# szemenyeim/DynEnv

Measured on AMD Instinct MI355X. Metric: agent-steps/s, higher is better.
Workload: dtype f64

## Files before the change

### dynenv_amd/csrc/driving_kernels.hip

```cpp
#include "driving_dev.h"

__constant__ DrvConst C;

#include "driving_host.h"

struct DrvMailbox {
  double p1x[DRV_NS][2], p1y[DRV_NS][2], p2x[DRV_NS][2], p2y[DRV_NS][2], nx[DRV_NS], ny[DRV_NS];
  int hash[DRV_NS][2], count[DRV_NS], flag[DRV_NS];
};
struct DrvObsStage {
  float carRow[DRV_MAXA][8];
  float goal[DRV_MAXA][2];
  float shared[DRV_MAXO * 4 + DRV_MAXP * 2 + DRV_LANE_ROWS * 5];
};
#ifdef DRV_PROFILE
#define DRV_PROF(...) __VA_ARGS__
#else
#define DRV_PROF(...)
#endif
#define DRV_CLIST 128
struct __align__(16) DrvLds {
  double px[DRV_NB], py[DRV_NB], vx[DRV_NB], vy[DRV_NB], ang[DRV_NB], w[DRV_NB], vbx[DRV_NB], vby[DRV_NB], wb[DRV_NB];
  double minv[DRV_NB], iinv[DRV_NB];
  double rc[16], rs[16], rotAng[16];
  double dirx[16], diry[16], prevx[16], prevy[16], goalx[16], goaly[16];
  double cosRel0[16];
  double dprev[16];
  double cmass[16], cpower[16], chx[16], chy[16];
  double aabb[DRV_MAXA][4];
  int flags[DRV_NB], moving[DRV_NB];
  double ox[DRV_MAXO], oy[DRV_MAXO];
  int s_pair[DRV_NS], s_meta[DRV_NS], s_hash0[DRV_NS], s_hash1[DRV_NS];
  double s_jn0[DRV_NS], s_jt0[DRV_NS], s_jn1[DRV_NS], s_jt1[DRV_NS];
  double rewAcc[16], posAcc[16];
  int lastCand[64];
  int stepErr;
  unsigned char act[16];
  int still[DRV_NB];
  unsigned short clist[DRV_CLIST];
  int clistN;
  int sLvMeta;
  unsigned long long sActive;
  unsigned char sLevel[DRV_NS];
  union {
    DrvMailbox mb;
    DrvObsStage ob;
  } u;
};

static_assert(sizeof(DrvLds) <= 10240, "16 one-wave workgroups per CU - one residency round of 4096 environments on 256 CUs - need <= 160 KB / 16 of LDS each");
__shared__ DrvLds g_L;


#define CF_FIN(f) (((f) >> 4) & 1)
#define CF_CRASHED(f) (((f) >> 5) & 1)
#define CF_FRIC(f) (((f) >> 6) & 1)
#define CF_LP(f) (((f) >> 8) & 7)
#define CF_SET_LP(f, lp) (((f) & ~(7 << 8)) | ((lp) << 8))
#define CF_CRASH_BITS ((1 << 4) | (1 << 5) | (1 << 6))
#define PF_ROAD(f) ((f)&1)
#define PF_SIDE(f) (((f) >> 1) & 1)
#define PF_DEAD(f) (((f) >> 2) & 1)
#define PF_CROSSING(f) (((f) >> 3) & 1)
#define PF_BEGIN(f) (((f) >> 4) & 1)
#define PF_SPEED(f) (((f) >> 8) & 15)

#define DRV_COS_PI_2 6.123233995736766e-17
template <int R>
struct RoadK;
template <>
struct RoadK<0> {
  static constexpr double p0x = 875.0, p0y = 0.0, dirx = 0.0, diry = 1.0, lat = 2.0 * 35.0 + 5.0, length = 1000.0;
  static constexpr double dirAngle = 1.5707963267948966, cosDir0 = DRV_COS_PI_2, nx = -1.0, ny = DRV_COS_PI_2;
};
template <>
struct RoadK<1> {
  static constexpr double p0x = 0.0, p0y = 500.0, dirx = 1.0, diry = 0.0, lat = 1.0 * 35.0 + 5.0, length = 1750.0;
  static constexpr double dirAngle = 0.0, cosDir0 = 1.0, nx = DRV_COS_PI_2, ny = 1.0;
};

struct CarK {
  static constexpr double carMass0 = 1200.0, carMass1 = 1800.0, carMass2 = 3500.0, carMass3 = 5000.0;
  static constexpr double carHx0 = 10.0, carHx1 = 15.0, carHx2 = 20.0, carHx3 = 25.0;
  static constexpr double carHy0 = 5.0, carHy1 = 6.0, carHy2 = 7.0, carHy3 = 8.0;
  static constexpr double carPower0 = 3.0, carPower1 = 4.0, carPower2 = 3.0, carPower3 = 4.0;
  static constexpr double carInertia0 = 50000.0, carInertia1 = 156600.0, carInertia2 = 0x1.ff8e555555555p+18, carInertia3 = 0x1.185ad55555555p+20;
  static constexpr double pedMass = 90.0, pedInertia = 90.0 * (0.5 * (0.0 * 0.0 + 5.0 * 5.0) + 0.0);
};

template <int R>
DE_DEV int road_pos(V2 point, double cosRel) {
  V2 pt = vsub(point, v2(RoadK<R>::p0x, RoadK<R>::p0y));
  double dist = vcross(v2(RoadK<R>::dirx, RoadK<R>::diry), pt);
  if (dm_abs(dist) >= RoadK<R>::lat) return LP_OffRoad;
  int pos = LP_OverRoad;
  double dirDist = vdot(v2(RoadK<R>::dirx, RoadK<R>::diry), pt);
  if (dirDist >= -10.0 && dirDist <= RoadK<R>::length + 10.0) {
    double relAngle = cosRel * dist;
    pos = relAngle < 0.0 ? LP_InRightLane : LP_InOpposingLane;
  }
  return pos;
}

DE_DEV bool drv_is_off_road(V2 point) {
  int position = LP_OffRoad;
  int rp = road_pos<0>(point, RoadK<0>::cosDir0);
  if (rp < position) position = rp;
  rp = road_pos<1>(point, RoadK<1>::cosDir0);
  if (rp < position) position = rp;
  return position >= LP_OverRoad;
}
DE_DEV bool drv_is_out(V2 p) { return p.x <= 0.0 || p.y <= 0.0 || p.x >= DRV_W || p.y >= DRV_H; }

DE_DEV void apply_friction(double& vx, double& vy, double& w, double m, double friction, double rotFriction,
                           double spin) {
  vx = vx * 1.0 + (0.0 + 0.0) * DE_DT;
  vy = vy * 1.0 + (0.0 + 0.0) * DE_DT;
  w = w * 1.0 + 0.0;
  double factor = friction * m;
// ... 256 lines not shown
  b.w = dm_fma(b.iinv, dms_cross(r.x, r.y, j.x, j.y), b.w);
}
DE_DEV void apply_bias_impulse(BodyV& b, V2 j, V2 r) {
  b.vb = v2(dm_fma(j.x, b.minv, b.vb.x), dm_fma(j.y, b.minv, b.vb.y));
  b.wb = dm_fma(b.iinv, dms_cross(r.x, r.y, j.x, j.y), b.wb);
}
DE_DEV double bias_rel_n(const BodyV& a, const BodyV& b, V2 r1, V2 r2, V2 n) {
  const V2 vb1 = v2(dms_point_vx(a.vb.x, r1.y, a.wb), dms_point_vy(a.vb.y, r1.x, a.wb));
  const V2 vb2 = v2(dms_point_vx(b.vb.x, r2.y, b.wb), dms_point_vy(b.vb.y, r2.x, b.wb));
  return vdot_f(vsub(vb2, vb1), n);
}

#define STD_NORM_X (0.5 / (DRV_W + 100.0))
#define STD_NORM_Y (0.5 / (DRV_H + 100.0))
#define STD_NORM_W (1.0 / 15.0)
#define STD_NORM_H (1.0 / 25.0)
DE_DEV double normalize_obs(double pt, double nf, double mean) { return ((pt * nf) - mean) * 2.0 * 1.0; }

DE_DEV float obs_self_or_car(const DrvObsStage& O, int A, int a, int ff) {
  if (ff < 6) return O.carRow[a][ff];
  if (ff < 8) return O.goal[a][ff - 6];
  if (ff == 8) return O.carRow[a][6];
  int c = (ff - 9) / 7, kk = (ff - 9) - c * 7;
  c += (c >= a);
  return O.carRow[c][kk];
}

DE_OOL void write_full_obs_ool(int lane, int A, int nPed, int nObst, int obs_dim, float* __restrict__ out) {
  DrvLds& L = g_L;
  DrvObsStage& O = L.u.ob;
  __syncthreads();
  if (lane < A) {
    int f = L.flags[lane];
    O.carRow[lane][0] = (float)normalize_obs(L.px[lane], STD_NORM_X, 0.0);
    O.carRow[lane][1] = (float)normalize_obs(L.py[lane], STD_NORM_Y, 0.0);
    O.carRow[lane][2] = (float)L.rc[lane];
    O.carRow[lane][3] = (float)L.rs[lane];
    O.carRow[lane][4] = (float)normalize_obs(L.chy[lane], STD_NORM_W, 0.5);
    O.carRow[lane][5] = (float)normalize_obs(L.chx[lane], STD_NORM_H, 0.5);
    O.carRow[lane][6] = (float)CF_FIN(f);
    O.goal[lane][0] = (float)normalize_obs(L.goalx[lane], STD_NORM_X, 0.0);
    O.goal[lane][1] = (float)normalize_obs(L.goaly[lane], STD_NORM_Y, 0.0);
  }
  if (lane >= DRV_SLOT_PED && lane < DRV_SLOT_PED + DRV_MAXP) {
    int k = lane - DRV_SLOT_PED;
    bool on = k < nPed;
    O.shared[DRV_MAXO * 4 + 2 * k + 0] = on ? (float)normalize_obs(L.px[lane], STD_NORM_X, 0.0) : 0.0f;
    O.shared[DRV_MAXO * 4 + 2 * k + 1] = on ? (float)normalize_obs(L.py[lane], STD_NORM_Y, 0.0) : 0.0f;
  }
  if (lane < DRV_MAXO) {
    bool on = lane < nObst;
    O.shared[4 * lane + 0] = on ? (float)normalize_obs(L.ox[lane], STD_NORM_X, 0.0) : 0.0f;
    O.shared[4 * lane + 1] = on ? (float)normalize_obs(L.oy[lane], STD_NORM_Y, 0.0) : 0.0f;
    O.shared[4 * lane + 2] = on ? (float)normalize_obs(10.0, STD_NORM_W, 0.5) : 0.0f;
    O.shared[4 * lane + 3] = on ? (float)normalize_obs(10.0, STD_NORM_H, 0.5) : 0.0f;
  }
  if (lane < DRV_LANE_ROWS * 5) O.shared[DRV_MAXO * 4 + DRV_MAXP * 2 + lane] = C.laneRows[lane];
  __syncthreads();
  const int carsEnd = 9 + (A - 1) * 7;
  if (((carsEnd | obs_dim) & 3) == 0) {
    for (int f = lane; f < carsEnd; f += DE_WAVE) {
      const bool own = f < 9;
      const int p = own ? 0 : (f - 9) / 7, col = own ? (f < 6 ? f : (f == 8 ? 6 : f - 6)) : (f - 9) - p * 7;
      const bool fromGoal = f == 6 || f == 7;
      for (int a = 0; a < A; ++a) {
        const int k = own ? a : p + (p >= a ? 1 : 0);
        out[(size_t)a * obs_dim + f] = fromGoal ? O.goal[a][col] : O.carRow[k][col];
      }
    }
    const int nvec = (obs_dim - carsEnd) >> 2;
    for (int q = lane; q < nvec; q += DE_WAVE) {
      const float4 v = *reinterpret_cast<const float4*>(&O.shared[q << 2]);
      for (int a = 0; a < A; ++a) *reinterpret_cast<float4*>(out + (size_t)a * obs_dim + carsEnd + (q << 2)) = v;
    }
  } else {
    for (int idx = lane; idx < A * obs_dim; idx += DE_WAVE) {
      int a = idx / obs_dim, ff = idx - a * obs_dim;
      out[idx] = ff < carsEnd ? obs_self_or_car(O, A, a, ff) : O.shared[ff - carsEnd];
    }
  }
  __syncthreads();
}

DE_DEV void load_env(const DrvState& S, DrvLds& L, int e, int lane, int A, int nPed, int nObst, uint64_t occ) {
  const size_t E = (size_t)S.E;
  const int bl = lane & (DRV_NB - 1), cl = lane & 15, ol = lane < DRV_MAXO ? lane : DRV_MAXO - 1, sl = lane < DRV_NS ? lane : DRV_NS - 1;
  const double* b = S.body + (size_t)e * DRV_NB + bl;
  const double g_px = b[BF_PX * E * DRV_NB], g_py = b[BF_PY * E * DRV_NB], g_vx = b[BF_VX * E * DRV_NB], g_vy = b[BF_VY * E * DRV_NB];
  const double g_ang = b[BF_ANG * E * DRV_NB], g_w = b[BF_W * E * DRV_NB];
  const double g_vbx = b[BF_VBX * E * DRV_NB], g_vby = b[BF_VBY * E * DRV_NB], g_wb = b[BF_WB * E * DRV_NB];
  const int g_f = S.flags[(size_t)e * DRV_NB + bl], g_aux = S.aux[(size_t)e * DRV_NB + bl];
  const double* c = S.carx + (size_t)e * 16 + cl;
  const double g_prevx = c[CF_PREVX * E * 16], g_prevy = c[CF_PREVY * E * 16], g_gx = c[CF_GOALX * E * 16], g_gy = c[CF_GOALY * E * 16];
  const double g_dirx = c[CF_DIRX * E * 16], g_diry = c[CF_DIRY * E * 16];
  const double g_ox = S.obst[(size_t)e * DRV_MAXO + ol], g_oy = S.obst[E * DRV_MAXO + (size_t)e * DRV_MAXO + ol];
  int g_pair = 0xFFFF, g_meta = 0, g_h0 = 0, g_h1 = 0;
  double g_jn0 = 0.0, g_jt0 = 0.0, g_jn1 = 0.0, g_jt1 = 0.0;
  if (occ != 0ull) {
    const size_t o = (size_t)e * DRV_NS + sl;
    g_pair = S.s_pair[o]; g_meta = S.s_meta[o];
    g_h0 = (int)S.s_hash[o]; g_h1 = (int)S.s_hash[E * DRV_NS + o];
    g_jn0 = S.s_imp[o]; g_jt0 = S.s_imp[E * DRV_NS + o]; g_jn1 = S.s_imp[2 * E * DRV_NS + o]; g_jt1 = S.s_imp[3 * E * DRV_NS + o];
  }
  if (lane < DRV_NB) {
    const bool used = lane < A || (lane >= DRV_SLOT_PED && lane < DRV_SLOT_PED + nPed);
    L.px[lane] = used ? g_px : 0.0; L.py[lane] = used ? g_py : 0.0;
    L.vx[lane] = used ? g_vx : 0.0; L.vy[lane] = used ? g_vy : 0.0;
    const double ang = used ? g_ang : 0.0;
    L.ang[lane] = ang; L.w[lane] = used ? g_w : 0.0;
    L.vbx[lane] = used ? g_vbx : 0.0; L.vby[lane] = used ? g_vby : 0.0;
    L.wb[lane] = used ? g_wb : 0.0;
    const int f = used ? g_f : 0;
    L.flags[lane] = f;
    L.moving[lane] = used ? g_aux : 0;
    const int ty = f & 3;
#define DRV_BY_TYPE(ARR) (ty == 3 ? CarK::ARR##3 : (ty == 2 ? CarK::ARR##2 : (ty == 1 ? CarK::ARR##1 : CarK::ARR##0)))
    double minv = 0.0, iinv = 0.0;
    if (lane < A) { minv = 1.0 / DRV_BY_TYPE(carMass); iinv = 1.0 / DRV_BY_TYPE(carInertia); }
    else if (used) { minv = 1.0 / CarK::pedMass; iinv = 1.0 / CarK::pedInertia; }
    L.minv[lane] = minv; L.iinv[lane] = iinv;
    if (lane < 16) { L.rc[lane] = 1.0; L.rs[lane] = 0.0; L.rotAng[lane] = 0.0; }
    if (lane < A) {
      L.dirx[lane] = g_dirx; L.diry[lane] = g_diry;
      L.prevx[lane] = g_prevx; L.prevy[lane] = g_prevy; L.goalx[lane] = g_gx; L.goaly[lane] = g_gy;
      L.dprev[lane] = vlen(vsub(v2(g_prevx, g_prevy), v2(g_gx, g_gy)));
      L.cmass[lane] = DRV_BY_TYPE(carMass); L.cpower[lane] = DRV_BY_TYPE(carPower);
      L.chx[lane] = DRV_BY_TYPE(carHx); L.chy[lane] = DRV_BY_TYPE(carHy);
      car_refresh_rot(L, lane, ang);
    }
#undef DRV_BY_TYPE
  }
  if (lane < DRV_MAXO) {
    L.ox[lane] = lane < nObst ? g_ox : 0.0;
    L.oy[lane] = lane < nObst ? g_oy : 0.0;
  }
  if (lane < DRV_NS) {
    const bool on = (occ >> lane) & 1ull;
    L.s_pair[lane] = on ? g_pair : 0xFFFF;
    L.s_meta[lane] = on ? g_meta : 0;
    L.s_hash0[lane] = on ? g_h0 : 0; L.s_hash1[lane] = on ? g_h1 : 0;
    L.s_jn0[lane] = on ? g_jn0 : 0.0; L.s_jt0[lane] = on ? g_jt0 : 0.0;
    L.s_jn1[lane] = on ? g_jn1 : 0.0; L.s_jt1[lane] = on ? g_jt1 : 0.0;
  }
}

DE_DEV void store_env(const DrvState& S, const DrvLds& L, int e, int lane, int A, int nPed, uint64_t occ) {
  const size_t E = (size_t)S.E;
  if (lane < A || (lane >= DRV_SLOT_PED && lane < DRV_SLOT_PED + nPed)) {
    double* b = S.body + (size_t)e * DRV_NB + lane;
    b[BF_PX * E * DRV_NB] = L.px[lane]; b[BF_PY * E * DRV_NB] = L.py[lane]; b[BF_VX * E * DRV_NB] = L.vx[lane];
    b[BF_VY * E * DRV_NB] = L.vy[lane]; b[BF_ANG * E * DRV_NB] = L.ang[lane]; b[BF_W * E * DRV_NB] = L.w[lane];
    b[BF_VBX * E * DRV_NB] = L.vbx[lane]; b[BF_VBY * E * DRV_NB] = L.vby[lane]; b[BF_WB * E * DRV_NB] = L.wb[lane];
    S.flags[(size_t)e * DRV_NB + lane] = L.flags[lane];
    if (lane < A) {
      double* c = S.carx + (size_t)e * 16 + lane;
      c[CF_DIRX * E * 16] = L.dirx[lane]; c[CF_DIRY * E * 16] = L.diry[lane];
      c[CF_PREVX * E * 16] = L.prevx[lane]; c[CF_PREVY * E * 16] = L.prevy[lane];
    } else {
      S.aux[(size_t)e * DRV_NB + lane] = L.moving[lane];
    }
  }
  if (lane < DRV_NS && ((occ >> lane) & 1ull)) {
    size_t o = (size_t)e * DRV_NS + lane;
    S.s_pair[o] = L.s_pair[lane]; S.s_meta[o] = L.s_meta[lane];
    S.s_hash[o] = (uint32_t)L.s_hash0[lane]; S.s_hash[E * DRV_NS + o] = (uint32_t)L.s_hash1[lane];
    S.s_imp[o] = L.s_jn0[lane]; S.s_imp[E * DRV_NS + o] = L.s_jt0[lane];
    S.s_imp[2 * E * DRV_NS + o] = L.s_jn1[lane]; S.s_imp[3 * E * DRV_NS + o] = L.s_jt1[lane];
  }
}

DE_DEV bool cb_begin(DrvLds& L, int i, int j, int lane) {
  const double v1x = L.vx[i], v1y = L.vy[i];
  const int f1 = L.flags[i];
  if (j < DRV_SLOT_PED) {
    const double v2x = L.vx[j], v2y = L.vy[j];
    const int f2 = L.flags[j];
    const int crashed1 = CF_CRASHED(f1), crashed2 = CF_CRASHED(f2), pos1 = CF_LP(f1), pos2 = CF_LP(f2);
    const double v1len = vlen(v2(v1x, v1y)), v2len = vlen(v2(v2x, v2y));
    const double v1l = v1len / 5.0, v2l = v2len / 5.0;
    double r1 = L.rewAcc[i], r2 = L.rewAcc[j];
    if (!crashed1) r1 -= v1l;
    if (!crashed2) r2 -= v2l;
    if (pos1 != LP_InRightLane && !crashed1) r1 -= v1l;
    if (pos2 != LP_InRightLane && !crashed2) r2 -= v2l;
    if (pos1 == LP_InRightLane && pos2 == LP_InRightLane) {
      V2 dp = v2(L.px[i] - L.px[j], L.py[i] - L.py[j]);
      double adp = dev_atan2(dp.y, dp.x);
      if (v1len > 1.0 && dev_cos(adp - dev_atan2(v1y, v1x)) < -0.4 && !crashed1) r1 -= v1l;
      if (v2len > 1.0 && dev_cos(adp - dev_atan2(v2y, v2x)) > 0.4 && !crashed2) r2 -= v2l;
    }
    if (lane == i) { L.rewAcc[i] = r1; L.flags[i] = f1 | CF_CRASH_BITS; }
    if (lane == j) { L.rewAcc[j] = r2; L.flags[j] = f2 | CF_CRASH_BITS; }
    return true;
  } else if (j < DRV_SLOT_OBST) {
    const double v1l = vlen(v2(v1x, v1y));
    if (v1l > 1.0) {
      V2 dp = v2(L.px[i] - L.px[j], L.py[i] - L.py[j]);
      if (lane == j) {
        L.moving[j] = 0; L.vx[j] = 0.0; L.vy[j] = 0.0; L.flags[j] = L.flags[j] | (1 << 2);
      }
      if (dev_cos(dev_atan2(dp.y, dp.x) - dev_atan2(v1y, v1x)) < -0.4 && !CF_FIN(f1)) {
        if (lane == i) { L.flags[i] = f1 | CF_CRASH_BITS; L.rewAcc[i] = L.rewAcc[i] - v1l / 5.0; }
      }
      return true;
    }
    return false;
  } else {
    if (lane == i) {
      if (!CF_FIN(f1)) L.rewAcc[i] = L.rewAcc[i] - vlen(v2(v1x, v1y)) / 5.0;
      L.flags[i] = f1 | CF_CRASH_BITS;
    }
    return true;
  }
}

DE_DEV void arb_warm_start(BodyV& a, BodyV& b, V2 n, const V2* r1, const V2* r2, const double* jn, const double* jt,
                           int count) {
#pragma unroll
  for (int c = 0; c < 2; ++c) {
    if (c == 0 || count > 1) {
      V2 j = vrotate_f(n, v2(jn[c], jt[c]));
      j = vmul(j, 1.0);
      apply_impulse(a, vneg(j), r1[c]);
      apply_impulse(b, j, r2[c]);
    }
  }
// ... 758 lines not shown
            const V2 nv = vmul(vmul(dir, (double)PF_SPEED(f)), (double)speed);
            vx = nv.x; vy = nv.y;
          } else if (isOffRoad) {
            crossing = 0; beginc = 0;
          }
        }
        L.moving[lane] = moving;
        L.flags[lane] = PEDF_PACK(PF_ROAD(f), side, 0, crossing, beginc, PF_SPEED(f));
        L.vx[lane] = vx; L.vy[lane] = vy;
      }
    }

DRV_PROF(const unsigned long long Q3 = __builtin_amdgcn_s_memtime();)
    double bl = 0.0, bb = 0.0, br = -1.0, bt = -1.0;
    bool live = false;
    int sj = 3;
    if (isBody) {
      const double npx = px + (vx + vbx) * DE_DT, npy = py + (vy + vby) * DE_DT, nang = ang + (w + wb) * DE_DT;
      const bool still = !turned && vx == 0.0 && vy == 0.0 && w == 0.0 && vbx == 0.0 && vby == 0.0 && wb == 0.0;
      L.px[lane] = npx; L.py[lane] = npy; L.ang[lane] = nang;
      const bool frozen = !turned && vx == 0.0 && vy == 0.0 && w == 0.0 && npx == px && npy == py && nang == ang;
      sj = (still ? 1 : 0) | (frozen ? 2 : 0);
      L.still[lane] = sj;
      live = true;
      if (isCar) {
        if (nang != rotAngv) { const CarRot cr = car_refresh_rot<true>(L, lane, nang); rcv = cr.c; rsv = cr.s; }
        if (!aabbValid || !frozen) {
          BoxW bw;
          box_world(bw, v2(npx, npy), rcv, rsv, chx, chy);
          double l = INFINITY, r = -INFINITY, b = INFINITY, t = -INFINITY;
#pragma unroll
          for (int k = 0; k < 4; ++k) {
            l = fmin_cp(l, bw.v[k].x); r = fmax_cp(r, bw.v[k].x); b = fmin_cp(b, bw.v[k].y); t = fmax_cp(t, bw.v[k].y);
          }
          bl = l - 0.0; bb = b - 0.0; br = r + 0.0; bt = t + 0.0;
          L.aabb[lane][0] = bl; L.aabb[lane][1] = bb; L.aabb[lane][2] = br; L.aabb[lane][3] = bt;
        } else {
          bl = L.aabb[lane][0]; bb = L.aabb[lane][1]; br = L.aabb[lane][2]; bt = L.aabb[lane][3];
        }
      } else {
        bl = npx - 5.0; bb = npy - 5.0; br = npx + 5.0; bt = npy + 5.0;
      }
    } else if (lane >= DRV_SLOT_OBST && lane < DRV_SLOT_BLD + 4) {
      live = lane >= DRV_SLOT_BLD || (lane - DRV_SLOT_OBST) < nObst;
      const V2 c = static_pos(L, lane);
      const double ex = lane >= DRV_SLOT_BLD ? 400.0 : 10.0, ey = lane >= DRV_SLOT_BLD ? 225.0 : 10.0;
      bl = -ex + c.x; br = ex + c.x; bb = -ey + c.y; bt = ey + c.y;
    }
    aabbValid = true;
    __syncthreads();
DRV_PROF(const unsigned long long Q4 = __builtin_amdgcn_s_memtime();)

    int cand = 0;
    bool candMoving = false, removed = false;
    int dirty = 0;
    {
      const int carStill = (int)(wave_ballot(isCar && (sj & 1)) & 0x3FFull);
      const int carFrozen = (int)(wave_ballot(isCar && (sj & 2)) & 0x3FFull);
#pragma unroll
      for (int i = 0; i < DRV_MAXA; ++i) {
        const double al = L.aabb[i][0], ab = L.aabb[i][1], ar = L.aabb[i][2], at = L.aabb[i][3];
        const bool hit = (al <= br) & (bl <= ar) & (ab <= bt) & (bb <= at);
        cand |= hit ? (1 << i) : 0;
      }
      {
        const int lim = lane < A ? lane : A;
        cand &= live ? ((1 << lim) - 1) : 0;
      }
      if (cand) candMoving = !(sj & 1) || (cand & ~carStill) != 0;
      const int clean = (lastCand >= 0 && (sj & 2)) ? (cand & lastCand & carFrozen) : 0;
      dirty = cand & ~clean;
      removed = lastCand < 0 || (lastCand & ~cand) != 0;
    }
  L.lastCand[lane] = cand;
DRV_PROF(if (lane == 0 && blockIdx.x < 4096) { unsigned long long* d = g_dbgl + blockIdx.x * 8; const unsigned long long Q5 = __builtin_amdgcn_s_memtime(); if (it == 0) { for (int k = 0; k < 8; ++k) d[k] = 0ull; } d[0] += Q1 - Q0; d[1] += Q2 - Q1; d[2] += Q3 - Q2; d[3] += Q4 - Q3; d[4] += Q5 - Q4; d[5] += Q5 - Q0; })
  DrvLightRet ret;
  ret.cand = cand; ret.dirty = dirty; ret.bits = (candMoving ? 1 : 0) | (removed ? 2 : 0) | (cand != lastCand ? 4 : 0);
  return ret;
}
DE_DEV unsigned drv_hw_simd_key() {
  const unsigned hw = (unsigned)__builtin_amdgcn_s_getreg(63492) , xcc = (unsigned)__builtin_amdgcn_s_getreg(63508) ;
  return ((xcc & 0xFu) << 16) | (hw & 0xFF30u);
}
DE_DEV int drv_launch_tick(const DrvState& S) { return S.tick_src ? uniform_i(__atomic_load_n(&S.iso[13], __ATOMIC_RELAXED)) : S.tick; }
DE_DEV int drv_launch_pv(const DrvState& S) { return S.tick_src ? uniform_i(__atomic_load_n(&S.iso[14], __ATOMIC_RELAXED)) : S.pv_par; }
DE_DEV int drv_iso_assign(const DrvState& S, int lane, int tick) {
  const int b = blockIdx.x, E = S.E;
  if (!S.iso_on) return b;
  const int buf = tick % 3;
  if (b == 0 && lane == 0) { const int nn = (tick + 2) % 3; S.iso[nn] = 0; S.iso[3 + nn] = 0; }
  if (S.iso_on == 3) return b;
  int K = uniform_i(S.iso[buf]);
  const int cap = S.iso_on == 1 ? DRV_ISO_MAX : DRV_ISO_LIST;
  K = K < cap ? K : cap;
  const int G = S.iso_on == 1 ? 4 * DRV_ISO_GROUPS : E;
  if (S.iso_on == 1) {
    if (b < G) { if (lane == 0) S.iso_hw[(size_t)(tick & 1) * (4 * DRV_ISO_GROUPS) + b] = drv_hw_simd_key(); }
    else if (b == G + 3 * DRV_ISO_MAX) {
      const unsigned* hw = S.iso_hw + (size_t)((tick + 1) & 1) * (4 * DRV_ISO_GROUPS);
      bool bad = false;
      for (int g = DRV_ISO_G0 + lane; g < DRV_ISO_G0 + DRV_ISO_GSPAN; g += 64) {
        const unsigned k0 = hw[g], k1 = hw[g + DRV_ISO_GROUPS], k2 = hw[g + 2 * DRV_ISO_GROUPS], k3 = hw[g + 3 * DRV_ISO_GROUPS];
        bad |= k0 == 0xFFFFFFFFu || k0 != k1 || k0 != k2 || k0 != k3;
      }
      const bool ok = wave_ballot(bad) == 0ull;
      if (lane == 0) {
        int cd = S.iso[12];
        if (!ok) cd = DRV_ISO_COOLDOWN; else if (cd > 0) cd -= 1;
        S.iso[12] = cd;
        S.iso[8 + (tick + 1) % 3] = (ok && cd == 0) ? 1 : 0;
        if (!ok && tick > 1) atomicAdd(&S.iso[11], 1);
      }
      return -1;
    }
    if (uniform_i(S.iso[8 + buf]) != 1) K = 0;
  }
  if (K == 0) return b < E ? b : -1;
  const int* H = S.iso + DRV_ISO_HDR + buf * DRV_ISO_LIST;
  int r;
  if (S.iso_on == 2) {
    if (b < K) return uniform_i(H[b]);
    r = b - K;
  } else if (b >= G) {
    const int d = b - G;
    if (d >= 3 * K) return -1;
    r = (G - 4 * K) + d;
  } else {
    const int g = b & (DRV_ISO_GROUPS - 1), pos = b / DRV_ISO_GROUPS;
    if ((unsigned)(g - DRV_ISO_G0) < (unsigned)K) {
      const int h = uniform_i(H[g - DRV_ISO_G0]);
      if (pos == 0) return h;
      int i = 0;
      for (; i < 96; ++i) {
        if (uniform_i(__atomic_load_n(&S.iso_done[h], __ATOMIC_RELAXED)) == tick) break;
        __builtin_amdgcn_s_sleep(127);
      }
      if (i >= 96 && lane == 0) atomicAdd(&S.iso[7], 1);
      return -1;
    }
    r = pos * (DRV_ISO_GROUPS - K) + (g < DRV_ISO_G0 ? g : g - K);
  }
  int h0 = 0x7FFFFFFF, h1 = h0, h2 = h0, h3 = h0;
  if (lane < K) h0 = H[lane];
  if (lane + 64 < K) h1 = H[lane + 64];
  if (lane + 128 < K) h2 = H[lane + 128];
  if (lane + 192 < K) h3 = H[lane + 192];
  int x = r;
  for (int it = 0; it <= DRV_ISO_LIST; ++it) {
    const int c = __popcll(wave_ballot(h0 <= x)) + __popcll(wave_ballot(h1 <= x)) + __popcll(wave_ballot(h2 <= x)) + __popcll(wave_ballot(h3 <= x));
    const int nx = r + c;
    if (nx == x) break;
    x = nx;
  }
  return x < E ? x : -1;
}
#ifndef DRV_ISO_MIN
#define DRV_ISO_MIN 300000
#endif
#ifndef DRV_ISO_PCT
#define DRV_ISO_PCT 75
#endif
DE_DEV void drv_iso_report(const DrvState& S, int e, int lane, unsigned long long t0, int tick) {
  if (!S.iso_on || lane != 0) return;
  const int cycles = (int)(__builtin_amdgcn_s_memtime() - t0);
  const int buf = tick % 3, nxt = (tick + 1) % 3;
  const int slowest = S.iso[3 + buf];
  if (cycles > DRV_ISO_MIN && cycles > (slowest / 100) * DRV_ISO_PCT) atomicMax(&S.iso[3 + nxt], cycles);
  if (S.iso_on == 3) return;
  if (slowest > DRV_ISO_MIN && cycles > (slowest / 100) * DRV_ISO_PCT) {
    const int k = atomicAdd(&S.iso[nxt], 1);
    if (k < DRV_ISO_LIST) S.iso[DRV_ISO_HDR + nxt * DRV_ISO_LIST + k] = e;
  }
  __atomic_store_n(&S.iso_done[e], tick, __ATOMIC_RELAXED);
}

template <bool PARTIAL>
DE_DEV void drv_step_body(const DrvState& S, const int* __restrict__ actions, float* __restrict__ obs, double* __restrict__ rewards,
                          uint8_t* __restrict__ dones, float* __restrict__ pobs, int pvNoise, double pvMagn) {
  const unsigned long long isoT0 = __builtin_amdgcn_s_memtime();
DRV_PROF(const unsigned long long KS = isoT0;)
  DrvLds& L = g_L;
  int lane = threadIdx.x;
  const int tick = drv_launch_tick(S);
  if (!S.tick_src && blockIdx.x == 0 && lane == 0) { S.iso[13] = S.tick; S.iso[14] = S.pv_par; }
  const int e = drv_iso_assign(S, lane, tick);
  if (e < 0) return;
DRV_PROF(if (lane < 8 && e < 4096) { g_dbgp[e * 8 + lane] = 0ull; g_dbgs[e * 8 + lane] = 0ull; })
  const int A = S.A;
  int* envi = S.envi + (size_t)e * EI_COUNT;
  int elapsed = uniform_i(envi[EI_ELAPSED]);
  int allFinished = uniform_i(envi[EI_ALLFIN]);
  const int nPed = uniform_i(envi[EI_NPED]);
  const int nObst = uniform_i(envi[EI_NOBST]);
  const uint32_t episode = (uint32_t)uniform_i(envi[EI_EPISODE]);
  uint64_t occ = (uint64_t)(uint32_t)uniform_i(envi[EI_OCC]);
  if (occ != 0ull) __builtin_amdgcn_s_setprio(3);
  else if (PARTIAL) __builtin_amdgcn_s_setprio(1);
  const uint32_t genv = (uint32_t)(S.env_id_offset + e);

  const bool isCar = lane < A;
  const bool isPed = lane >= DRV_SLOT_PED && lane < DRV_SLOT_PED + nPed;
  const bool isBody = isCar || isPed;
  const int g_act0 = actions[((size_t)e * A + (isCar ? lane : 0)) * 2 + 0], g_act1 = actions[((size_t)e * A + (isCar ? lane : 0)) * 2 + 1];
  const int g_lastCand = S.lastcand[(size_t)e * 64 + lane];
  load_env(S, L, e, lane, A, nPed, nObst, occ);

  {
    int act0 = isCar ? g_act0 : 1, act1 = isCar ? g_act1 : 1;
    const bool bad = (unsigned)act0 > 2u || (unsigned)act1 > 2u;
    if (bad) { act0 = 1; act1 = 1; }
    if (lane < 16) L.act[lane] = (unsigned char)(act0 | (act1 << 2));
    const bool anyBad = wave_ballot(bad) != 0ull;
    if (lane == 0) L.stepErr = anyBad ? 2 : 0;
  }
  int finishedAt = -1;
  if (lane < 16) { L.rewAcc[lane] = 0.0; L.posAcc[lane] = 0.0; }
  bool aabbValid = false;
  L.lastCand[lane] = g_lastCand;
  if (lane == 0) { L.clistN = -1; L.sActive = ~0ull; L.sLvMeta = 0; }
  bool inertAll = (uniform_i(envi[EI_PAD]) & 1) != 0;
  bool steadyAll = (uniform_i(envi[EI_PAD]) & 2) != 0;
  bool vbValid = (uniform_i(envi[EI_PAD]) & 4) != 0;
  int nFast = 0, nQuiet = 0, nContact = 0, nSlots = 0, nWhyCand = 0, nWhyMoving = 0, nWhyInert = 0, nSteady = 0, nLight = 0, nSplit = 0;
  __syncthreads();

DRV_PROF(const unsigned long long K0 = __builtin_amdgcn_s_memtime(); unsigned long long tPh1 = 0, tBroad = 0, tFast = 0, tCont = 0, tBook = 0;)
  bool lightOff = false;
  for (int it = 0; it < 10; ++it) {
    lane = fresh_lane();
DRV_PROF(const unsigned long long A0 = __builtin_amdgcn_s_memtime();)
    const DrvLightRet lr = drv_light_substep(it, lane, A, nPed, nObst, elapsed, (uint32_t)S.seed, (uint32_t)(S.seed >> 32), genv, episode,
                                             (vbValid ? 1 : 0) | (aabbValid ? 2 : 0));
    const int cand = lr.cand, dirty = lr.dirty;
    const bool candMoving = (lr.bits & 1) != 0, removed = (lr.bits & 2) != 0;
    aabbValid = true;
DRV_PROF(const unsigned long long A1 = A0;)
    const uint64_t anyCand = wave_ballot(cand != 0);
    const bool candChanged = wave_ballot((lr.bits & 4) != 0) != 0ull, anyMoving = wave_ballot(candMoving) != 0ull;
    if (candChanged && lane == 0) L.clistN = -1;
    const bool quiescent = inertAll && !candChanged && !anyMoving;
    const bool steadyOk = !quiescent && steadyAll && wave_ballot(removed) == 0ull;
    const bool anyDirty = wave_ballot(dirty != 0) != 0ull;
    bool replay = steadyOk && !anyDirty;
    const bool light = steadyOk && anyDirty && !lightOff;
    if (!(anyCand == 0ull && occ == 0ull) && !quiescent && !replay) { if (candChanged) nWhyCand++; else if (anyMoving) nWhyMoving++; else nWhyInert++; }

DRV_PROF(const unsigned long long A2 = __builtin_amdgcn_s_memtime(); bool tookContact = false;)
    if (anyCand == 0ull && occ == 0ull) nFast++; else if (quiescent) nQuiet++; else if (replay) nSteady++; else nContact++;
    nSlots += __popcll(occ);
    if ((anyCand == 0ull && occ == 0ull) || quiescent) {
      velocity_update_ool(A | (nPed << 8));
      if (anyCand == 0ull && occ == 0ull) steadyAll = false;
      vbValid = false;
    } else if (!replay) {
DRV_PROF(tookContact = true;)
      __builtin_amdgcn_s_setprio(3);
      ContactRet cr = drv_contact_path(lane, cand, dirty, light ? 1 : 0, A, A | (nPed << 8), occ);
      lane = fresh_lane();
      if (wave_ballot((cr.err & 1) != 0) != 0ull && lane == 0) L.stepErr |= 1;
      if (light && !(uniform_i(cr.err >> 3) & 1)) lightOff = true;
      if (uniform_i(cr.err >> 3) & 1) {
        replay = true; nLight++;
      } else {
        nSplit += uniform_i(cr.err >> 4) & 1;
        occ = uniform_u64(cr.occ);
        inertAll = (uniform_i(cr.err >> 1) & 1) != 0;
        steadyAll = (uniform_i(cr.err >> 2) & 1) != 0;
        vbValid = true;
      }
    }
    if (replay) {
      velocity_update_ool(A | (nPed << 8));
      vbValid = true;
    }
    __syncthreads();

DRV_PROF(const unsigned long long A3 = __builtin_amdgcn_s_memtime(); tPh1 += A1 - A0; tBroad += A2 - A1; if (tookContact) tCont += A3 - A2; else tFast += A3 - A2;)
    elapsed += 1;
    bool notDone = false;
    if (isCar) { int f = L.flags[lane]; notDone = !(CF_FIN(f) && !CF_CRASHED(f)); }
    const bool allFin = wave_ballot(notDone) == 0ull;
    if (!allFinished && allFin) {
      allFinished = 1;
      finishedAt = elapsed;
    }
  }
  lane = fresh_lane();
  const double teamReward = finishedAt >= 0 ? 0.0 + (double)(DRV_MAX_TIME - finishedAt) / 100.0 : 0.0;

DRV_PROF(const unsigned long long K1 = __builtin_amdgcn_s_memtime();)
  double* er = S.epr + (size_t)e * 16 + (isCar ? lane : 0);
  double* ep = S.epr + (size_t)S.E * 16 + (size_t)e * 16 + (isCar ? lane : 0);
  const double g_er = *er, g_ep = *ep;
  const int cl = lane < 10 ? lane : 0;
  const int g_cnt = envi[EI_N_FAST + cl];
  const int g_err = envi[EI_ERR];
  double rew = 0.0, posrew = 0.0;
  if (isCar) {
    rew = L.rewAcc[lane] + teamReward;
    posrew = L.posAcc[lane] + dm_max(0.0, teamReward);
    rewards[(size_t)e * A + lane] = rew;
  }
  if (lane == 0) {
    dones[e] = (uint8_t)(elapsed >= DRV_MAX_TIME);
    envi[EI_ELAPSED] = elapsed; envi[EI_ALLFIN] = allFinished; envi[EI_OCC] = (int)(uint32_t)occ;
    envi[EI_PAD] = (inertAll ? 1 : 0) | (steadyAll ? 2 : 0) | (vbValid ? 4 : 0);
  }
  const int errBits = uniform_i(L.stepErr);
  S.lastcand[(size_t)e * 64 + lane] = L.lastCand[lane];
  store_env(S, L, e, lane, A, nPed, occ);
  if (obs) write_full_obs_ool(lane, A, nPed, nObst, S.obs_dim, obs + (size_t)e * A * S.obs_dim);
  if (isCar) { *er = g_er + rew; *ep = g_ep + posrew; }
  {
    static_assert(EI_N_QUIET == EI_N_FAST + 1 && EI_N_CONTACT == EI_N_FAST + 2 && EI_N_SLOTS == EI_N_FAST + 3 && EI_N_WHY_CAND == EI_N_FAST + 4 &&
                  EI_N_WHY_MOVING == EI_N_FAST + 5 && EI_N_WHY_INERT == EI_N_FAST + 6 && EI_N_STEADY == EI_N_FAST + 7 && EI_N_LIGHT == EI_N_FAST + 8 && EI_N_SPLIT == EI_N_FAST + 9,
                  "the diagnostic counters are consecutive");
    const int add = lane == 0 ? nFast : lane == 1 ? nQuiet : lane == 2 ? nContact : lane == 3 ? nSlots : lane == 4 ? nWhyCand : lane == 5 ? nWhyMoving :
                    lane == 6 ? nWhyInert : lane == 7 ? nSteady : lane == 8 ? nLight : nSplit;
    if (lane < 10) envi[EI_N_FAST + lane] = g_cnt + add;
  }
  if (errBits && lane == 0) envi[EI_ERR] = g_err | errBits;
  int fusedAgents = !(PARTIAL && pobs) ? 0 : nContact >= DRV_DEFER_MIN_CONTACT ? 0 : (A < DRV_FUSED_AGENTS ? A : DRV_FUSED_AGENTS);
  int budget = 0;
  if (PARTIAL && pobs && S.iso_on >= 2) {
    const int slowest = uniform_i(S.iso[3 + tick % 3]);
    if (slowest > 0) {
      budget = (slowest / 100) * DRV_PV_DEADLINE_PCT - (int)(__builtin_amdgcn_s_memtime() - isoT0);
      fusedAgents = budget > 0 ? A : 0;
    }
  }
  drv_iso_report(S, e, fresh_lane(), isoT0, tick);
  if (PARTIAL && fusedAgents > 0) {
    __builtin_amdgcn_s_setprio(0);
    PvIn in;
    in.px = in.py = in.ang = in.ox = in.oy = in.gx = in.gy = 0.0; in.flags = 0;
    if (lane < DRV_NB && (lane < A || (lane >= DRV_SLOT_PED && lane < DRV_SLOT_PED + nPed))) {
      in.px = L.px[lane]; in.py = L.py[lane]; in.ang = L.ang[lane]; in.flags = L.flags[lane];
    }
    if (lane < nObst) { in.ox = L.ox[lane]; in.oy = L.oy[lane]; }
    if (lane < A) { in.gx = L.goalx[lane]; in.gy = L.goaly[lane]; }
    fusedAgents = drv_partial_obs_fused(in, S.seed, S.A, S.envi, S.env_id_offset, e, nPed | (nObst << 8), elapsed, episode, pvNoise | (fusedAgents << 8), pvMagn,
                                        pobs, budget);
  }
  if (PARTIAL && fresh_lane() == 0) {
    envi[EI_DEFER_OBS] = fusedAgents;
    if (pobs && fusedAgents < A) {
      const int pv = drv_launch_pv(S);
      const int k = atomicAdd(&S.pvq[16 * pv], 1);
      if (k < S.E) S.pvq[32 + pv * S.E + k] = e;
      else envi[EI_ERR] = envi[EI_ERR] | 4;
    }
  }
DRV_PROF(if (lane == 0 && e < 4096) { unsigned long long* d = g_dbgw + e * 12; const unsigned long long KE = __builtin_amdgcn_s_memtime(); d[0] = KE - KS; d[1] = nContact; d[2] = __popcll(occ); d[3] = nSteady + nQuiet; d[4] = K0 - KS; d[5] = tPh1; d[6] = tBroad; d[7] = tFast; d[8] = tCont; d[9] = (K1 - K0) - tPh1 - tBroad - tFast - tCont; d[10] = KE - K1; d[11] = ((unsigned long long)__builtin_amdgcn_s_getreg(63508) << 32) | (unsigned long long)__builtin_amdgcn_s_getreg(63492); })
}

extern "C" __global__ void drv_tick_advance_kernel(DrvState S, int flipPv) {
  if (threadIdx.x == 0 && blockIdx.x == 0) { S.iso[13] = (S.iso[13] + 1) % (3 * (1 << 28)); if (flipPv) S.iso[14] = S.iso[14] ^ 1; }
}

extern "C" __global__ void __launch_bounds__(64, DRV_WAVES_PER_SIMD)
drv_step_kernel(DrvState S, const int* __restrict__ actions, float* __restrict__ obs, double* __restrict__ rewards,
                uint8_t* __restrict__ dones) {
  drv_step_body<false>(S, actions, obs, rewards, dones, nullptr, 0, 0.0);
}
extern "C" __global__ void __launch_bounds__(64, DRV_WAVES_PER_SIMD)
drv_step_partial_kernel(DrvState S, const int* __restrict__ actions, double* __restrict__ rewards, uint8_t* __restrict__ dones,
                        float* __restrict__ pobs, int pvNoise, double pvMagn) {
  drv_step_body<true>(S, actions, nullptr, rewards, dones, pobs, pvNoise, pvMagn);
}

extern "C" __global__ void __launch_bounds__(64) drv_obs_kernel(DrvState S, float* __restrict__ obs) {
  DrvLds& L = g_L;
  const int e = blockIdx.x, lane = threadIdx.x, A = S.A;
  const int* envi = S.envi + (size_t)e * EI_COUNT;
  const int nPed = uniform_i(envi[EI_NPED]), nObst = uniform_i(envi[EI_NOBST]);
  load_env(S, L, e, lane, A, nPed, nObst, 0ull);
  write_full_obs_ool(lane, A, nPed, nObst, S.obs_dim, obs + (size_t)e * A * S.obs_dim);
}

DE_DEV void road_get_spot(const DrvRoad& r, int lane, int spot, V2& pos, double& angle) {
  int end = lane >= r.nLanes ? 1 : 0;
  V2 p = end ? r.p1 : r.p0;
  V2 spotDir = vmul(end ? vneg(r.dir) : r.dir, r.followDist);
  V2 laneDir = vmul(end ? r.normal : vneg(r.normal), r.width);
  double l = (double)(end ? lane - r.nLanes : lane) + 0.5;
  pos = vadd(vadd(p, vmul(laneDir, l)), vmul(spotDir, (double)spot));
  angle = dm_atan2(spotDir.y, spotDir.x);
}
DE_DEV V2 road_get_walk_spot(const DrvRoad& r, int side, double length, double width) {
  V2 w0 = r.walk[side][0], w1 = r.walk[side][1];
  V2 center = vadd(w0, vmul(vsub(w1, w0), length));
  double f = width * r.width;
  V2 off = vmul(vmul(r.normal, f), side ? 1.0 : -1.0);
  return vadd(center, off);
}

extern "C" __global__ void __launch_bounds__(64) drv_reset_kernel(DrvState S) {
  const int e = blockIdx.x * blockDim.x + threadIdx.x;
  if (e >= S.E) return;
  const size_t E = (size_t)S.E;
  const int A = S.A;
  int* envi = S.envi + (size_t)e * EI_COUNT;
  const uint32_t ep = (uint32_t)envi[EI_EPISODE];
  const uint32_t genv = (uint32_t)(S.env_id_offset + e);
  for (int k = 0; k < DRV_NB; ++k) {
    for (int f = 0; f < BF_COUNT; ++f) S.body[(size_t)f * E * DRV_NB + (size_t)e * DRV_NB + k] = 0.0;
    S.flags[(size_t)e * DRV_NB + k] = 0;
    S.aux[(size_t)e * DRV_NB + k] = 0;
  }
  for (int k = 0; k < 16; ++k) {
    for (int f = 0; f < CF_COUNT; ++f) S.carx[(size_t)f * E * 16 + (size_t)e * 16 + k] = 0.0;
    S.epr[(size_t)e * 16 + k] = 0.0;
    S.epr[E * 16 + (size_t)e * 16 + k] = 0.0;
  }
// ... 211 lines not shown
```

Measured before the change: 261.7 million.

## Batch kernel-entry global loads and broadcast iso header via readlane

The kernel prologue now issues every per-environment global load (envi words, actions, lastcand, body/car/obstacle/slot state) up front in one batch behind a sched_barrier, instead of many dependent uniform loads. Scalars are then pulled out with readlane. The iso scheduling header and work lists are loaded once per lane and broadcast, replacing repeated scalar global reads, and the slowest-time value is cached in LDS for later use. This aims to cut serialized load latency at wave start, at the cost of more live registers and loading slot data even when it is unoccupied.

Measured after the change: 260.5 million. No clear change (-0.4%).

```diff
diff --git a/dynenv_amd/csrc/driving_kernels.hip b/dynenv_amd/csrc/driving_kernels.hip
--- a/dynenv_amd/csrc/driving_kernels.hip
+++ b/dynenv_amd/csrc/driving_kernels.hip
@@ -35,6 +35,7 @@
   double rewAcc[16], posAcc[16];
   int lastCand[64];
   int stepErr;
+  int isoSlowest;
   unsigned char act[16];
   int still[DRV_NB];
   unsigned short clist[DRV_CLIST];
@@ -457,37 +458,41 @@
   __syncthreads();
 }
 
-DE_DEV void load_env(const DrvState& S, DrvLds& L, int e, int lane, int A, int nPed, int nObst, uint64_t occ) {
+struct DrvEnvLoads {
+  double px, py, vx, vy, ang, w, vbx, vby, wb, prevx, prevy, gx, gy, dirx, diry, ox, oy, jn0, jt0, jn1, jt1;
+  int f, aux, pair, meta, h0, h1;
+};
+DE_DEV DrvEnvLoads drv_env_loads(const DrvState& S, int e, int lane) {
   const size_t E = (size_t)S.E;
   const int bl = lane & (DRV_NB - 1), cl = lane & 15, ol = lane < DRV_MAXO ? lane : DRV_MAXO - 1, sl = lane < DRV_NS ? lane : DRV_NS - 1;
+  DrvEnvLoads g;
   const double* b = S.body + (size_t)e * DRV_NB + bl;
-  const double g_px = b[BF_PX * E * DRV_NB], g_py = b[BF_PY * E * DRV_NB], g_vx = b[BF_VX * E * DRV_NB], g_vy = b[BF_VY * E * DRV_NB];
-  const double g_ang = b[BF_ANG * E * DRV_NB], g_w = b[BF_W * E * DRV_NB];
-  const double g_vbx = b[BF_VBX * E * DRV_NB], g_vby = b[BF_VBY * E * DRV_NB], g_wb = b[BF_WB * E * DRV_NB];
-  const int g_f = S.flags[(size_t)e * DRV_NB + bl], g_aux = S.aux[(size_t)e * DRV_NB + bl];
+  g.px = b[BF_PX * E * DRV_NB]; g.py = b[BF_PY * E * DRV_NB]; g.vx = b[BF_VX * E * DRV_NB]; g.vy = b[BF_VY * E * DRV_NB];
+  g.ang = b[BF_ANG * E * DRV_NB]; g.w = b[BF_W * E * DRV_NB];
+  g.vbx = b[BF_VBX * E * DRV_NB]; g.vby = b[BF_VBY * E * DRV_NB]; g.wb = b[BF_WB * E * DRV_NB];
+  g.f = S.flags[(size_t)e * DRV_NB + bl]; g.aux = S.aux[(size_t)e * DRV_NB + bl];
   const double* c = S.carx + (size_t)e * 16 + cl;
-  const double g_prevx = c[CF_PREVX * E * 16], g_prevy = c[CF_PREVY * E * 16], g_gx = c[CF_GOALX * E * 16], g_gy = c[CF_GOALY * E * 16];
-  const double g_dirx = c[CF_DIRX * E * 16], g_diry = c[CF_DIRY * E * 16];
-  const double g_ox = S.obst[(size_t)e * DRV_MAXO + ol], g_oy = S.obst[E * DRV_MAXO + (size_t)e * DRV_MAXO + ol];
-  int g_pair = 0xFFFF, g_meta = 0, g_h0 = 0, g_h1 = 0;
-  double g_jn0 = 0.0, g_jt0 = 0.0, g_jn1 = 0.0, g_jt1 = 0.0;
-  if (occ != 0ull) {
-    const size_t o = (size_t)e * DRV_NS + sl;
-    g_pair = S.s_pair[o]; g_meta = S.s_meta[o];
-    g_h0 = (int)S.s_hash[o]; g_h1 = (int)S.s_hash[E * DRV_NS + o];
-    g_jn0 = S.s_imp[o]; g_jt0 = S.s_imp[E * DRV_NS + o]; g_jn1 = S.s_imp[2 * E * DRV_NS + o]; g_jt1 = S.s_imp[3 * E * DRV_NS + o];
-  }
+  g.prevx = c[CF_PREVX * E * 16]; g.prevy = c[CF_PREVY * E * 16]; g.gx = c[CF_GOALX * E * 16]; g.gy = c[CF_GOALY * E * 16];
+  g.dirx = c[CF_DIRX * E * 16]; g.diry = c[CF_DIRY * E * 16];
+  g.ox = S.obst[(size_t)e * DRV_MAXO + ol]; g.oy = S.obst[E * DRV_MAXO + (size_t)e * DRV_MAXO + ol];
+  const size_t o = (size_t)e * DRV_NS + sl;
+  g.pair = S.s_pair[o]; g.meta = S.s_meta[o];
+  g.h0 = (int)S.s_hash[o]; g.h1 = (int)S.s_hash[E * DRV_NS + o];
+  g.jn0 = S.s_imp[o]; g.jt0 = S.s_imp[E * DRV_NS + o]; g.jn1 = S.s_imp[2 * E * DRV_NS + o]; g.jt1 = S.s_imp[3 * E * DRV_NS + o];
+  return g;
+}
+DE_DEV void drv_env_fill(DrvLds& L, const DrvEnvLoads& g, int lane, int A, int nPed, int nObst, uint64_t occ) {
   if (lane < DRV_NB) {
     const bool used = lane < A || (lane >= DRV_SLOT_PED && lane < DRV_SLOT_PED + nPed);
-    L.px[lane] = used ? g_px : 0.0; L.py[lane] = used ? g_py : 0.0;
-    L.vx[lane] = used ? g_vx : 0.0; L.vy[lane] = used ? g_vy : 0.0;
-    const double ang = used ? g_ang : 0.0;
-    L.ang[lane] = ang; L.w[lane] = used ? g_w : 0.0;
-    L.vbx[lane] = used ? g_vbx : 0.0; L.vby[lane] = used ? g_vby : 0.0;
-    L.wb[lane] = used ? g_wb : 0.0;
-    const int f = used ? g_f : 0;
+    L.px[lane] = used ? g.px : 0.0; L.py[lane] = used ? g.py : 0.0;
+    L.vx[lane] = used ? g.vx : 0.0; L.vy[lane] = used ? g.vy : 0.0;
+    const double ang = used ? g.ang : 0.0;
+    L.ang[lane] = ang; L.w[lane] = used ? g.w : 0.0;
+    L.vbx[lane] = used ? g.vbx : 0.0; L.vby[lane] = used ? g.vby : 0.0;
+    L.wb[lane] = used ? g.wb : 0.0;
+    const int f = used ? g.f : 0;
     L.flags[lane] = f;
-    L.moving[lane] = used ? g_aux : 0;
+    L.moving[lane] = used ? g.aux : 0;
     const int ty = f & 3;
 #define DRV_BY_TYPE(ARR) (ty == 3 ? CarK::ARR##3 : (ty == 2 ? CarK::ARR##2 : (ty == 1 ? CarK::ARR##1 : CarK::ARR##0)))
     double minv = 0.0, iinv = 0.0;
@@ -496,9 +501,9 @@
     L.minv[lane] = minv; L.iinv[lane] = iinv;
     if (lane < 16) { L.rc[lane] = 1.0; L.rs[lane] = 0.0; L.rotAng[lane] = 0.0; }
     if (lane < A) {
-      L.dirx[lane] = g_dirx; L.diry[lane] = g_diry;
-      L.prevx[lane] = g_prevx; L.prevy[lane] = g_prevy; L.goalx[lane] = g_gx; L.goaly[lane] = g_gy;
-      L.dprev[lane] = vlen(vsub(v2(g_prevx, g_prevy), v2(g_gx, g_gy)));
+      L.dirx[lane] = g.dirx; L.diry[lane] = g.diry;
+      L.prevx[lane] = g.prevx; L.prevy[lane] = g.prevy; L.goalx[lane] = g.gx; L.goaly[lane] = g.gy;
+      L.dprev[lane] = vlen(vsub(v2(g.prevx, g.prevy), v2(g.gx, g.gy)));
       L.cmass[lane] = DRV_BY_TYPE(carMass); L.cpower[lane] = DRV_BY_TYPE(carPower);
       L.chx[lane] = DRV_BY_TYPE(carHx); L.chy[lane] = DRV_BY_TYPE(carHy);
       car_refresh_rot(L, lane, ang);
@@ -506,17 +511,21 @@
 #undef DRV_BY_TYPE
   }
   if (lane < DRV_MAXO) {
-    L.ox[lane] = lane < nObst ? g_ox : 0.0;
-    L.oy[lane] = lane < nObst ? g_oy : 0.0;
+    L.ox[lane] = lane < nObst ? g.ox : 0.0;
+    L.oy[lane] = lane < nObst ? g.oy : 0.0;
   }
   if (lane < DRV_NS) {
     const bool on = (occ >> lane) & 1ull;
-    L.s_pair[lane] = on ? g_pair : 0xFFFF;
-    L.s_meta[lane] = on ? g_meta : 0;
-    L.s_hash0[lane] = on ? g_h0 : 0; L.s_hash1[lane] = on ? g_h1 : 0;
-    L.s_jn0[lane] = on ? g_jn0 : 0.0; L.s_jt0[lane] = on ? g_jt0 : 0.0;
-    L.s_jn1[lane] = on ? g_jn1 : 0.0; L.s_jt1[lane] = on ? g_jt1 : 0.0;
-  }
+    L.s_pair[lane] = on ? g.pair : 0xFFFF;
+    L.s_meta[lane] = on ? g.meta : 0;
+    L.s_hash0[lane] = on ? g.h0 : 0; L.s_hash1[lane] = on ? g.h1 : 0;
+    L.s_jn0[lane] = on ? g.jn0 : 0.0; L.s_jt0[lane] = on ? g.jt0 : 0.0;
+    L.s_jn1[lane] = on ? g.jn1 : 0.0; L.s_jt1[lane] = on ? g.jt1 : 0.0;
+  }
+}
+
+DE_DEV void load_env(const DrvState& S, DrvLds& L, int e, int lane, int A, int nPed, int nObst, uint64_t occ) {
+  drv_env_fill(L, drv_env_loads(S, e, lane), lane, A, nPed, nObst, occ);
 }
 
 DE_DEV void store_env(const DrvState& S, const DrvLds& L, int e, int lane, int A, int nPed, uint64_t occ) {
@@ -1441,15 +1450,30 @@
   const unsigned hw = (unsigned)__builtin_amdgcn_s_getreg(63492) , xcc = (unsigned)__builtin_amdgcn_s_getreg(63508) ;
   return ((xcc & 0xFu) << 16) | (hw & 0xFF30u);
 }
-DE_DEV int drv_launch_tick(const DrvState& S) { return S.tick_src ? uniform_i(__atomic_load_n(&S.iso[13], __ATOMIC_RELAXED)) : S.tick; }
 DE_DEV int drv_launch_pv(const DrvState& S) { return S.tick_src ? uniform_i(__atomic_load_n(&S.iso[14], __ATOMIC_RELAXED)) : S.pv_par; }
-DE_DEV int drv_iso_assign(const DrvState& S, int lane, int tick) {
+static_assert(DRV_ISO_LIST == 4 * DE_WAVE && DRV_ISO_MAX <= DRV_ISO_LIST, "a list is four words per lane");
+DE_DEV int drv_sel3(int k, int a, int b, int c) { return k == 0 ? a : (k == 1 ? b : c); }
+DE_DEV int drv_iso_assign(const DrvState& S, int lane, int& tick, int& slowest) {
   const int b = blockIdx.x, E = S.E;
+  tick = S.tick; slowest = 0;
+  if (!S.iso_on && !S.tick_src) return b;
+  const int* iso = S.iso;
+  const int hdr = iso[lane & (DRV_ISO_HDR - 1)];
+  int la0 = 0, la1 = 0, la2 = 0, la3 = 0, lb0 = 0, lb1 = 0, lb2 = 0, lb3 = 0, lc0 = 0, lc1 = 0, lc2 = 0, lc3 = 0;
+  if (S.iso_on == 1 || S.iso_on == 2) {
+    const int* l = iso + DRV_ISO_HDR + lane;
+    la0 = l[0]; la1 = l[64]; la2 = l[128];
+    lb0 = l[DRV_ISO_LIST]; lb1 = l[DRV_ISO_LIST + 64]; lb2 = l[DRV_ISO_LIST + 128];
+    lc0 = l[2 * DRV_ISO_LIST]; lc1 = l[2 * DRV_ISO_LIST + 64]; lc2 = l[2 * DRV_ISO_LIST + 128];
+    if (S.iso_on == 2 || DRV_ISO_MAX > 3 * DE_WAVE) { la3 = l[192]; lb3 = l[DRV_ISO_LIST + 192]; lc3 = l[2 * DRV_ISO_LIST + 192]; }
+  }
+  if (S.tick_src) tick = __builtin_amdgcn_readlane(hdr, 13);
   if (!S.iso_on) return b;
   const int buf = tick % 3;
+  slowest = bcast_i(hdr, 3 + buf);
   if (b == 0 && lane == 0) { const int nn = (tick + 2) % 3; S.iso[nn] = 0; S.iso[3 + nn] = 0; }
   if (S.iso_on == 3) return b;
-  int K = uniform_i(S.iso[buf]);
+  int K = bcast_i(hdr, buf);
   const int cap = S.iso_on == 1 ? DRV_ISO_MAX : DRV_ISO_LIST;
   K = K < cap ? K : cap;
   const int G = S.iso_on == 1 ? 4 * DRV_ISO_GROUPS : E;
@@ -1463,8 +1487,8 @@
         bad |= k0 == 0xFFFFFFFFu || k0 != k1 || k0 != k2 || k0 != k3;
       }
       const bool ok = wave_ballot(bad) == 0ull;
+      int cd = __builtin_amdgcn_readlane(hdr, 12);
       if (lane == 0) {
-        int cd = S.iso[12];
         if (!ok) cd = DRV_ISO_COOLDOWN; else if (cd > 0) cd -= 1;
         S.iso[12] = cd;
         S.iso[8 + (tick + 1) % 3] = (ok && cd == 0) ? 1 : 0;
@@ -1472,13 +1496,15 @@
       }
       return -1;
     }
-    if (uniform_i(S.iso[8 + buf]) != 1) K = 0;
+    if (bcast_i(hdr, 8 + buf) != 1) K = 0;
   }
   if (K == 0) return b < E ? b : -1;
-  const int* H = S.iso + DRV_ISO_HDR + buf * DRV_ISO_LIST;
+  int h0 = drv_sel3(buf, la0, lb0, lc0), h1 = drv_sel3(buf, la1, lb1, lc1), h2 = drv_sel3(buf, la2, lb2, lc2), h3 = drv_sel3(buf, la3, lb3, lc3);
+  h0 = lane < K ? h0 : 0x7FFFFFFF; h1 = lane + 64 < K ? h1 : 0x7FFFFFFF; h2 = lane + 128 < K ? h2 : 0x7FFFFFFF; h3 = lane + 192 < K ? h3 : 0x7FFFFFFF;
+  const auto entry = [&](int k) { const int c = k >> 6; return bcast_i(c == 0 ? h0 : (c == 1 ? h1 : (c == 2 ? h2 : h3)), k & 63); };
   int r;
   if (S.iso_on == 2) {
-    if (b < K) return uniform_i(H[b]);
+    if (b < K) return entry(b);
     r = b - K;
   } else if (b >= G) {
     const int d = b - G;
@@ -1487,7 +1513,7 @@
   } else {
     const int g = b & (DRV_ISO_GROUPS - 1), pos = b / DRV_ISO_GROUPS;
     if ((unsigned)(g - DRV_ISO_G0) < (unsigned)K) {
-      const int h = uniform_i(H[g - DRV_ISO_G0]);
+      const int h = entry(g - DRV_ISO_G0);
       if (pos == 0) return h;
       int i = 0;
       for (; i < 96; ++i) {
@@ -1499,11 +1525,6 @@
     }
     r = pos * (DRV_ISO_GROUPS - K) + (g < DRV_ISO_G0 ? g : g - K);
   }
-  int h0 = 0x7FFFFFFF, h1 = h0, h2 = h0, h3 = h0;
-  if (lane < K) h0 = H[lane];
-  if (lane + 64 < K) h1 = H[lane + 64];
-  if (lane + 128 < K) h2 = H[lane + 128];
-  if (lane + 192 < K) h3 = H[lane + 192];
   int x = r;
   for (int it = 0; it <= DRV_ISO_LIST; ++it) {
     const int c = __popcll(wave_ballot(h0 <= x)) + __popcll(wave_ballot(h1 <= x)) + __popcll(wave_ballot(h2 <= x)) + __popcll(wave_ballot(h3 <= x));
@@ -1519,11 +1540,10 @@
 #ifndef DRV_ISO_PCT
 #define DRV_ISO_PCT 75
 #endif
-DE_DEV void drv_iso_report(const DrvState& S, int e, int lane, unsigned long long t0, int tick) {
+DE_DEV void drv_iso_report(const DrvState& S, int e, int lane, unsigned long long t0, int tick, int slowest) {
   if (!S.iso_on || lane != 0) return;
   const int cycles = (int)(__builtin_amdgcn_s_memtime() - t0);
-  const int buf = tick % 3, nxt = (tick + 1) % 3;
-  const int slowest = S.iso[3 + buf];
+  const int nxt = (tick + 1) % 3;
   if (cycles > DRV_ISO_MIN && cycles > (slowest / 100) * DRV_ISO_PCT) atomicMax(&S.iso[3 + nxt], cycles);
   if (S.iso_on == 3) return;
   if (slowest > DRV_ISO_MIN && cycles > (slowest / 100) * DRV_ISO_PCT) {
@@ -1540,29 +1560,34 @@
 DRV_PROF(const unsigned long long KS = isoT0;)
   DrvLds& L = g_L;
   int lane = threadIdx.x;
-  const int tick = drv_launch_tick(S);
   if (!S.tick_src && blockIdx.x == 0 && lane == 0) { S.iso[13] = S.tick; S.iso[14] = S.pv_par; }
-  const int e = drv_iso_assign(S, lane, tick);
+  int tick, isoSlowest;
+  const int e = drv_iso_assign(S, lane, tick, isoSlowest);
   if (e < 0) return;
 DRV_PROF(if (lane < 8 && e < 4096) { g_dbgp[e * 8 + lane] = 0ull; g_dbgs[e * 8 + lane] = 0ull; })
   const int A = S.A;
   int* envi = S.envi + (size_t)e * EI_COUNT;
-  int elapsed = uniform_i(envi[EI_ELAPSED]);
-  int allFinished = uniform_i(envi[EI_ALLFIN]);
-  const int nPed = uniform_i(envi[EI_NPED]);
-  const int nObst = uniform_i(envi[EI_NOBST]);
-  const uint32_t episode = (uint32_t)uniform_i(envi[EI_EPISODE]);
-  uint64_t occ = (uint64_t)(uint32_t)uniform_i(envi[EI_OCC]);
+  const int g_envi = envi[lane < EI_COUNT ? lane : 0];
+  const int al = lane < A ? lane : 0;
+  const int g_act0 = actions[((size_t)e * A + al) * 2 + 0], g_act1 = actions[((size_t)e * A + al) * 2 + 1];
+  const int g_lastCand = S.lastcand[(size_t)e * 64 + lane];
+  const DrvEnvLoads g_env = drv_env_loads(S, e, lane);
+  __builtin_amdgcn_sched_barrier(0);
+  static_assert(EI_COUNT <= DE_WAVE, "one word of envi per lane");
+  int elapsed = __builtin_amdgcn_readlane(g_envi, EI_ELAPSED);
+  int allFinished = __builtin_amdgcn_readlane(g_envi, EI_ALLFIN);
+  const int nPed = __builtin_amdgcn_readlane(g_envi, EI_NPED);
+  const int nObst = __builtin_amdgcn_readlane(g_envi, EI_NOBST);
+  const uint32_t episode = (uint32_t)__builtin_amdgcn_readlane(g_envi, EI_EPISODE);
+  uint64_t occ = (uint64_t)(uint32_t)__builtin_amdgcn_readlane(g_envi, EI_OCC);
+  const int carried = __builtin_amdgcn_readlane(g_envi, EI_PAD);
   if (occ != 0ull) __builtin_amdgcn_s_setprio(3);
   else if (PARTIAL) __builtin_amdgcn_s_setprio(1);
   const uint32_t genv = (uint32_t)(S.env_id_offset + e);
 
   const bool isCar = lane < A;
-  const bool isPed = lane >= DRV_SLOT_PED && lane < DRV_SLOT_PED + nPed;
-  const bool isBody = isCar || isPed;
-  const int g_act0 = actions[((size_t)e * A + (isCar ? lane : 0)) * 2 + 0], g_act1 = actions[((size_t)e * A + (isCar ? lane : 0)) * 2 + 1];
-  const int g_lastCand = S.lastcand[(size_t)e * 64 + lane];
-  load_env(S, L, e, lane, A, nPed, nObst, occ);
+  drv_env_fill(L, g_env, lane, A, nPed, nObst, occ);
+  if (lane == 0) L.isoSlowest = isoSlowest;
 
   {
     int act0 = isCar ? g_act0 : 1, act1 = isCar ? g_act1 : 1;
@@ -1577,9 +1602,9 @@
   bool aabbValid = false;
   L.lastCand[lane] = g_lastCand;
   if (lane == 0) { L.clistN = -1; L.sActive = ~0ull; L.sLvMeta = 0; }
-  bool inertAll = (uniform_i(envi[EI_PAD]) & 1) != 0;
-  bool steadyAll = (uniform_i(envi[EI_PAD]) & 2) != 0;
-  bool vbValid = (uniform_i(envi[EI_PAD]) & 4) != 0;
+  bool inertAll = (carried & 1) != 0;
+  bool steadyAll = (carried & 2) != 0;
+  bool vbValid = (carried & 4) != 0;
   int nFast = 0, nQuiet = 0, nContact = 0, nSlots = 0, nWhyCand = 0, nWhyMoving = 0, nWhyInert = 0, nSteady = 0, nLight = 0, nSplit = 0;
   __syncthreads();
 
@@ -1682,13 +1707,13 @@
   int fusedAgents = !(PARTIAL && pobs) ? 0 : nContact >= DRV_DEFER_MIN_CONTACT ? 0 : (A < DRV_FUSED_AGENTS ? A : DRV_FUSED_AGENTS);
   int budget = 0;
   if (PARTIAL && pobs && S.iso_on >= 2) {
-    const int slowest = uniform_i(S.iso[3 + tick % 3]);
+    const int slowest = uniform_i(L.isoSlowest);
     if (slowest > 0) {
       budget = (slowest / 100) * DRV_PV_DEADLINE_PCT - (int)(__builtin_amdgcn_s_memtime() - isoT0);
       fusedAgents = budget > 0 ? A : 0;
     }
   }
-  drv_iso_report(S, e, fresh_lane(), isoT0, tick);
+  drv_iso_report(S, e, fresh_lane(), isoT0, tick, L.isoSlowest);
   if (PARTIAL && fusedAgents > 0) {
     __builtin_amdgcn_s_setprio(0);
     PvIn in;
```
